# Opendigitalradio/ODR-AudioEnc

Hardware: AMD Instinct MI355X
Metric: real-time stereo DAB MP2 streams sustained (frames/s) @128 kbps/48 kHz (higher is better)
Workload: dtype f64; 1 GPU; 4096 streams/GPU x 48 kHz stereo (mode 's') x 128 kbps, psy 1, full encode (BASELINE configs[1]), 32 frames/stream/step; streams_per_gpu=4096, parallelism=streams sharded over 1 GPU(s), no data-path collective

## Files before the change

odr-audioenc_amd/csrc/mp2_psy13.h:

```cpp
#ifndef MP2_WAVE_PARTS
#error "include mp2_wave.h"
#endif

#define TL_LOGTAB(db) ((const uint64_t *)((db) + 1002))
TL_FN double tl_power_db(double e, const uint64_t *lt)
{
    return 10 * tlm_log10_pn(__builtin_fmax(e, 1E-20), lt) + TL_POWERNORM;
}
TL_FN double tl_power_db_main(double e, const uint64_t *lt, bool *near1)
{
    return 10 * tlm_log10_main_pn(__builtin_fmax(e, 1E-20), lt, near1) + TL_POWERNORM;
}
#define TL_DEFER(w) ((uint16_t *)(w).cinfo)
TL_FN void tl_power_near1(TlPsyLds &w, int pos0, int cnt)
{
    TL_LANES_BEGIN
    if (lane < cnt) {
        const int i = TL_DEFER(w)[pos0 + lane];
        const double e = w.u.fft[TL_EX(i)];
        TL_PX(w)[i] = 10 * tlm_log10_near1_pn(__builtin_fmax(e, 1E-20)) + TL_POWERNORM;
    }
    TL_LANES_END
}
#define TL_POWER_DEFER(w, flag, line_expr, ndef) do { \
// ... 245 lines not shown
    }
    TL_LANES_END
    int nlist = 0;
    if (!any_erased) {
        nlist = nconf;
        TL_LANES_BEGIN
        for (int i = lane; i < nconf; i += 64) w.tlist[i] = (int16_t)i;
        TL_LANES_END
    } else {
        PV(int, nx0); PV(int, nx1);
        TL_LANES_BEGIN L(nx0) = w.conf_nxt[lane]; L(nx1) = w.conf_nxt[64 + lane < TL_TONE_MAX ? 64 + lane : 0]; TL_LANES_END
        int i = nconf ? 0 : TL_LAST, guard = 0;
        while (i != TL_LAST && i != TL_STOP && guard++ < TL_TONE_MAX) {
            w.tlist[nlist++] = (int16_t)i;
            i = i < 64 ? TL_READLANE_I32(nx0, i) : TL_READLANE_I32(nx1, i - 64);
        }
        TL_SYNC();
    }
    TL_STAMP(sp, 3);

    const int nbands = C->p1_ncb - 1;
    {
        double *vt = w.u.fft, *vp = px;
        int nvalid = 0;
        PA(uint32_t, linfo, 8); PA(double, lrw, 8);
        TL_LANES_BEGIN
#ifndef TL_EMULATE
#pragma unroll
#endif
        for (int c8 = 0; c8 < 8; c8++) { L(linfo)[c8] = C->p1_lineinfo[64 * c8 + lane]; L(lrw)[c8] = C->p1_linerw[64 * c8 + lane]; }
        TL_LANES_END
#ifndef TL_EMULATE
#pragma unroll
#endif
        for (int base = 0; base < (TL_EXP_LEVEL >= 4 ? 0 : 512); base += 64) {
            PV(bool, ok); PV(double, tv); PV(double, pvv); PV(int, bnd);
            TL_LANES_BEGIN
            const int j = base + lane;
            const uint32_t info = L(linfo)[base >> 6];
            const int lo = (int)((info >> 8) & 0xfffu), hi = (int)(info >> 20);
            bool v = false; double t = 0, p = 0;
            if (info) {
                p = px[j];
                v = w.ptype[j] != TL_T_TONE && p != TL_DBMIN;
                t = tl_div_by(1073741824 * energy[TL_EX(j)] * (double)(j - lo), (double)(hi - lo), L(lrw)[base >> 6]);
            }
            L(ok) = v; L(tv) = t; L(pvv) = p; L(bnd) = (info && j == lo) ? (int)(info & 0xffu) : -1;
            TL_LANES_END
            const uint64_t m = TL_BALLOT(ok);
            TL_LANES_BEGIN
            const int pos = nvalid + __builtin_popcountll(m & ((1ull << lane) - 1ull));
            if (L(bnd) >= 0) w.bandoff[L(bnd)] = (int16_t)pos;
            if (L(ok)) { vt[pos] = L(tv); vp[pos] = L(pvv); }
            TL_LANES_END
            nvalid += __builtin_popcountll(m);
        }
        w.bandoff[nbands] = (int16_t)nvalid;
        TL_SYNC();
    }
    TlPsy1Ch r;
    r.nconf = nconf; r.nlist = nlist;
    r.dead_head = nconf > 0 && ((w.conf_c[0] >> 13) & 1);
    TL_DBG_TONES(nconf, r.dead_head); TL_DBG_CAND(ncand);
    return r;
}

TL_FN void tl_psy1_weights2(TlPsyLds &w, int nbands, PARG(int, r0), PARG(int, r1), PARG(double, wt))
{
    TL_LANES_BEGIN
    double weight = 0.0;
    const int band = lane & 31;
    if (band < nbands) {
        const bool second = lane >= 32;
        const double *vt = second ? w.u.fft : TL_PX(w);
        const int i0 = second ? (int)w.bandoff[band] : L(r0), i1 = second ? (int)w.bandoff[band + 1] : L(r1);
        int i = i0;
        for (; i + 16 <= i1; i += 16) {
            double t[16];
#ifndef TL_EMULATE
#pragma unroll
#endif
            for (int q = 0; q < 16; q++) t[q] = vt[i + q];
#ifndef TL_EMULATE
#pragma unroll
#endif
            for (int q = 0; q < 16; q++) weight += t[q];
        }
        for (; i < i1; i++) weight += vt[i];
    }
    L(wt) = weight;
    TL_LANES_END
}

TL_FN void tl_psy1_chain(TlPsyLds &w, const double *TL_RESTRICT db, int nbands, PARG(double, bsum), PARG(double, wt))
{
    TL_LANES_BEGIN
    double sum = TL_DBMIN, weight = 0.0;
    if (lane < nbands) {
        const double *vt = w.u.fft, *vp = TL_PX(w);
        const int i0 = w.bandoff[lane], i1 = w.bandoff[lane + 1];
        int i = i0;
        for (; i + 4 <= i1; i += 4) {
            const double p0 = vp[i], p1 = vp[i + 1], p2 = vp[i + 2], p3 = vp[i + 3];
            const double t0 = vt[i], t1 = vt[i + 1], t2 = vt[i + 2], t3 = vt[i + 3];
            sum = tl_add_db(db, p0, sum); weight += t0;
            sum = tl_add_db(db, p1, sum); weight += t1;
            sum = tl_add_db(db, p2, sum); weight += t2;
            sum = tl_add_db(db, p3, sum); weight += t3;
        }
        for (; i < i1; i++) { sum = tl_add_db(db, vp[i], sum); weight += vt[i]; }
    }
    L(bsum) = sum; L(wt) = weight;
    TL_LANES_END
}

TL_FN void tl_psy1_chain2(TlPsyLds &w, const double *TL_RESTRICT db, int nbands, PARG(int, r0), PARG(int, r1), PARG(double, bsum))
{
    TL_LANES_BEGIN
    double sum = TL_DBMIN;
    const int band = lane & 31;
    if (band < nbands) {
        const bool second = lane >= 32;
        const double *vp = second ? TL_PX(w) : w.u.fft;
        const int i0 = second ? (int)w.bandoff[band] : L(r0), i1 = second ? (int)w.bandoff[band + 1] : L(r1);
        int i = i0;
        for (; i + 8 <= i1; i += 8) {
            double p[8];
#ifndef TL_EMULATE
#pragma unroll
#endif
            for (int q = 0; q < 8; q++) p[q] = vp[i + q];
#ifndef TL_EMULATE
#pragma unroll
#endif
            for (int q = 0; q < 8; q++) sum = tl_add_db(db, p[q], sum);
        }
        for (; i + 4 <= i1; i += 4) {
            const double p0 = vp[i], p1 = vp[i + 1], p2 = vp[i + 2], p3 = vp[i + 3];
            sum = tl_add_db(db, p0, sum); sum = tl_add_db(db, p1, sum); sum = tl_add_db(db, p2, sum); sum = tl_add_db(db, p3, sum);
        }
        for (; i < i1; i++) sum = tl_add_db(db, vp[i], sum);
    }
    L(bsum) = sum;
    TL_LANES_END
}

TL_FN void tl_psy1_limits(const TlConfig *TL_RESTRICT C, int nbands, PARG(int, blo), PARG(int, bhi))
{
    TL_LANES_BEGIN
    const int b = lane < nbands ? lane : 0;
    L(blo) = C->p1_cbound[b]; L(bhi) = C->p1_cbound[b + 1];
    TL_LANES_END
}
TL_FN void tl_psy1_centres(TlPsyLds &w, int nbands, PARG(double, bsum), PARG(double, wt), PARG(int, blo), PARG(int, bhi))
{
    TL_LANES_BEGIN
    if (lane < nbands) {
        const int lo = L(blo), hi = L(bhi);
        const double sum = L(bsum), weight = L(wt);
        int centre;
        if (sum <= TL_DBMIN) centre = (hi + lo) / 2;
        else {
            double index = weight * tlm_pow10_sl(-0.1 * sum);
            centre = lo + (int)(index * (double)(hi - lo));
        }
        centre = centre < 1 ? 1 : centre > 510 ? 510 : centre;
        if (w.ptype[centre] == TL_T_TONE) { if (w.ptype[centre + 1] == TL_T_TONE) centre++; else centre--; }
        w.nsum[lane] = sum; w.ncentre[lane] = (int16_t)centre;
    }
    TL_LANES_END
}

TL_FN void tl_psy1_thresholds(TlPsyLds &w, const double *TL_RESTRICT db, const TlConfig *TL_RESTRICT C, int ch, int ntone, int nnoise, PARGA(double, rec, 4), long long *sp)
{
    TL_STAMP(sp, 5);
    TL_PRIO2(TL_PS_THR);

    TL_DBG_DUMP("psy1", ch, ntone, nnoise, TL_MK_X(w), TL_MK_BARK(w));
    const int sub = C->p1_sub;
    PV(double, tb0); PV(double, tb1); PV(double, th0); PV(double, th1); PV(int, mmn); PV(int, mmj);
    TL_LANES_BEGIN
    {
        const int k0 = 1 + 2 * lane, k1 = k0 + 1;
        const int q0 = k0 < sub ? k0 : 0, q1 = k1 < sub ? k1 : q0;
        L(tb0) = C->p1_bark[q0]; L(tb1) = C->p1_bark[q1]; L(th0) = C->p1_hear[q0]; L(th1) = C->p1_hear[q1];
        L(mmn) = C->p1_mm_n[lane & 31]; L(mmj) = C->p1_mm_j0[lane & 31];
    }
    TL_LANES_END
    TL_LANES_BEGIN
    for (int t = lane; t < ntone + nnoise; t += 64) tl_masker_consts(TL_MK4(w), TL_MK_X(w), TL_MK_BARK(w), t, t < ntone);
    TL_LANES_END
    const bool srt = ntone < 128 && nnoise < 64 && tl_maskers_sorted(TL_MK_BARK(w), ntone, nnoise);
    for (int base = 1; base < (TL_EXP_LEVEL >= 1 ? 0 : sub); base += 128) {
        TL_LANES_BEGIN
        const int k0 = base + 2 * lane, k1 = k0 + 1;
        const bool h0 = k0 < sub, h1 = k1 < sub;
        if (h0) {
            double bk0 = L(tb0), bk1 = L(tb1), hr0 = L(th0), hr1 = L(th1);
            if (base != 1) {
                bk0 = C->p1_bark[k0]; bk1 = C->p1_bark[h1 ? k1 : k0]; hr0 = C->p1_hear[k0]; hr1 = C->p1_hear[h1 ? k1 : k0];
            }
            const double blo = (bk0 < bk1 ? bk0 : bk1) - 8.0, bhi = (bk0 < bk1 ? bk1 : bk0) + 3.0;
            const TlMasker *mk = TL_MK4(w);
            const int nm = ntone + nnoise;
            int a0, a1, b0, b1;
            if (srt) tl_mask_spans_sorted<64, 32>(TL_MK_BARK(w), ntone, nnoise, blo, bhi, a0, a1, b0, b1);
            else tl_mask_spans(mk, nm, ntone, blo, bhi, a0, a1, b0, b1);
            double x0 = TL_DBMIN, x1 = TL_DBMIN;
            const int nt = a1 >= a0 ? a1 - a0 + 1 : 0, cnt = nt + (b1 >= b0 ? b1 - b0 + 1 : 0);
            int t = nt ? a0 : b0;
            TL_DBG_WALK(ch, lane, cnt);
            const TlMaskK kk = tl_mask_consts();
            for (int i = 0; i < cnt; i += 2) {
                const int tA = t, tB = tA == a1 ? b0 : tA + 1;
                t = tB == a1 ? b0 : tB + 1;
                const TlMasker *pA = &mk[tA & (TL_MASKER_MAX - 1)], *pB = &mk[tB & (TL_MASKER_MAX - 1)];
                const double bA = pA->bark, avA = pA->av, bB = pB->bark, avB = pB->av;
                const bool two = i + 1 < cnt;
                const double mA0 = tl_mask_term_w(pA, bA - bk0, avA, kk.far_hi), mA1 = tl_mask_term_w(pA, bA - bk1, avA, kk.far_hi);
                const double mB0 = tl_mask_term_w(pB, bB - bk0, avB, kk.far_hi, two), mB1 = tl_mask_term_w(pB, bB - bk1, avB, kk.far_hi, two);
                tl_add_db2_k(db, kk.k1000, x0, mA0, x1, mA1);
                tl_add_db2_k(db, kk.k1000, x0, mB0, x1, mB1);
            }
            TL_LTG(w)[k0] = tl_add_db(db, C->br_per_ch < 96 ? hr0 : hr0 - 12.0, x0);
            if (h1) TL_LTG(w)[k1] = tl_add_db(db, C->br_per_ch < 96 ? hr1 : hr1 - 12.0, x1);
        }
        TL_LANES_END
    }
    TL_STAMP(sp, 6);

    TL_LANES_BEGIN
    if (lane < C->sblimit) {
        double m;
        int n = L(mmn), j0 = L(mmj);
        if (n == 0) m = C->p1_hear[sub - 1];
        else {
            m = tl_min_rows(TL_LTG(w), j0, n, 0.0, true);
        }
        L(rec)[2 + ch] = m;
    } else if (lane < 32) L(rec)[2 + ch] = 0.0;
    TL_LANES_END
}

TL_FN void tl_psy1_back(TlPsyLds &w, const double *TL_RESTRICT db, const TlConfig *TL_RESTRICT C, int ch, const TlPsy1Ch &st, PARGA(double, rec, 4), long long *sp, bool stamp4 = true)
{
    const int nbands = C->p1_ncb - 1, nlist = st.nlist;
    int ntone = 0, nnoise = 0;
    if (stamp4) TL_STAMP(sp, 4);
    if (TL_EXP_LEVEL >= 2) { tl_psy1_thresholds(w, db, C, ch, 0, 0, rec, sp); return; }
    PV(int, ncen); PV(double, nlev); PV(int, nsh); PV(int, nsl); PV(bool, ontone);
    TL_LANES_BEGIN
    L(ncen) = lane < nbands ? (int)w.ncentre[lane] : -1 - lane;
    const double v = lane < nbands ? w.nsum[lane] : 0.0;
    L(nlev) = v; L(nsh) = (int)(uint32_t)(tl_d2u(v) >> 32); L(nsl) = (int)(uint32_t)tl_d2u(v);
    L(ontone) = lane < nbands && w.ptype[L(ncen)] == TL_T_TONE;
    TL_LANES_END
    const bool centre_on_tone = TL_BALLOT(ontone) != 0ull;
    PV(bool, shared_c);
    uint8_t *cmark = (uint8_t *)w.cinfo;
    TL_LANES_BEGIN if (lane < nbands) cmark[L(ncen)] = (uint8_t)lane; TL_LANES_END
    TL_LANES_BEGIN L(shared_c) = lane < nbands && cmark[L(ncen)] != (uint8_t)lane; TL_LANES_END
    if (TL_BALLOT(shared_c) != 0ull)
        for (int b = 1; b < nbands; b++) {
            const int cb = TL_READLANE_I32(ncen, b);
            const double vb = tl_u2d(((uint64_t)(uint32_t)TL_READLANE_I32(nsh, b) << 32) | (uint32_t)TL_READLANE_I32(nsl, b));
            TL_LANES_BEGIN if (lane < b && L(ncen) == cb) L(nlev) = vb; TL_LANES_END
        }

    {
        PV(double, nbk0); PV(double, nhear0);
        TL_LANES_BEGIN
        const int c0 = lane < nbands ? L(ncen) : 1;
        L(nbk0) = C->p1_lbark[c0]; L(nhear0) = C->p1_lhear[c0];
        TL_LANES_END
        for (int base = 0; base < nlist; base += 64) {
            PV(bool, keep); PV(double, kx); PV(double, kb); PV(int, tline); PV(int, tcc); PV(double, tbk); PV(double, thr);
            TL_LANES_BEGIN
            double x = 0; int c = -1000 - lane, cc = 0;
            if (base + lane < nlist) { const int ti = w.tlist[base + lane]; cc = w.conf_c[ti]; c = cc & 511; x = w.tone_x[ti]; }
            L(kx) = x; L(tline) = c; L(tcc) = cc;
            L(tbk) = C->p1_lbark[c < 0 ? 0 : c]; L(thr) = C->p1_lhear[c < 0 ? 0 : c];
            TL_LANES_END
            if (centre_on_tone)
                for (int b = 0; b < nbands; b++) {
                    const int cb = TL_READLANE_I32(ncen, b);
                    const double vb = tl_u2d(((uint64_t)(uint32_t)TL_READLANE_I32(nsh, b) << 32) | (uint32_t)TL_READLANE_I32(nsl, b));
                    TL_LANES_BEGIN if (L(tline) == cb) L(kx) = vb; TL_LANES_END
                }
            TL_LANES_BEGIN
            bool kp = false; double bk = 0;
            if (base + lane < nlist) {
                bk = L(tbk);
                kp = !((L(tcc) >> 13) & 1) && !(L(kx) < L(thr));
            }
            L(keep) = kp; L(kb) = bk;
            TL_LANES_END
            const uint64_t m = TL_BALLOT(keep);
            TL_LANES_BEGIN
            if ((m >> lane) & 1ull) {
                const int pos = ntone + __builtin_popcountll(m & ((1ull << lane) - 1ull));
                TL_MK_X(w)[pos] = L(kx); TL_MK_BARK(w)[pos] = L(kb);
            }
            TL_LANES_END
            ntone += __builtin_popcountll(m);
        }
        {
            PV(bool, closep);
            TL_LANES_BEGIN
            bool cl = false;
            for (int q = 1 + lane; q < ntone; q += 64) cl = cl || (TL_MK_BARK(w)[q] - TL_MK_BARK(w)[q - 1] < 0.5);
            L(closep) = cl;
            TL_LANES_END
            if (TL_BALLOT(closep) != 0ull) {
                int n = 0;
                double xi = TL_MK_X(w)[0], bi = TL_MK_BARK(w)[0];
                for (int q = 1; q < ntone; q++) {
                    const double xn = TL_MK_X(w)[q], bn = TL_MK_BARK(w)[q];
                    if (bn - bi < 0.5) {
                        if (xn > xi) { xi = xn; bi = bn; }
                    } else { TL_MK_X(w)[n] = xi; TL_MK_BARK(w)[n] = bi; n++; xi = xn; bi = bn; }
                }
                TL_MK_X(w)[n] = xi; TL_MK_BARK(w)[n] = bi; n++;
                ntone = n;
                TL_SYNC();
            }
        }
        PV(bool, keepn); PV(double, nx); PV(double, nb);
        TL_LANES_BEGIN
        bool kp = false; double x = 0, bk = 0;
        if (lane < nbands) {
            x = L(nlev); bk = L(nbk0);
            kp = !(x < L(nhear0));
        }
        L(keepn) = kp; L(nx) = x; L(nb) = bk;
        TL_LANES_END
        const uint64_t mn = TL_BALLOT(keepn);
        TL_LANES_BEGIN
        if ((mn >> lane) & 1ull) {
            const int pos = ntone + __builtin_popcountll(mn & ((1ull << lane) - 1ull));
            TL_MK_X(w)[pos] = L(nx); TL_MK_BARK(w)[pos] = L(nb);
        }
        TL_LANES_END
        nnoise = __builtin_popcountll(mn);
    }
    tl_psy1_thresholds(w, db, C, ch, ntone, nnoise, rec, sp);
}

TL_FN void tl_psy1_deadhead(TlPsyLds &w, const double *TL_RESTRICT db, const TlConfig *TL_RESTRICT C, int ch, const TlPsy1Ch &st, PARGA(double, rec, 4), long long *sp)
{
    const int nbands = C->p1_ncb - 1, nconf = st.nconf;
    const uint8_t *map = C->p1_map;
    double *px = TL_PX(w);
    int ntone = 0, nnoise = 0;
    TL_STAMP(sp, 4);
    {
        TL_LANES_BEGIN
        for (int j = lane; j < 520; j += 64) px[j] = TL_DBMIN;
        TL_LANES_END
        TL_LANES_BEGIN
        for (int i = lane; i < nconf; i += 64) { const int cc = w.conf_c[i]; if (!((cc >> 13) & 1)) px[cc & 511] = w.tone_x[i]; }
        TL_LANES_END
        TL_DBG_DUMP("deadhead", ch, 0, 0, px, px);
        int16_t *pnext = (int16_t *)w.cinfo;
        TL_LANES_BEGIN
        for (int i = lane; i < 512; i += 64) pnext[i] = TL_STOP;
        TL_LANES_END
        TL_LANES_BEGIN
        for (int i = lane; i < nconf; i += 64) {
            const int nx = w.conf_nxt[i];
            pnext[w.conf_c[i] & 511] = (int16_t)(nx >= 0 ? (w.conf_c[nx] & 511) : nx);
        }
        TL_LANES_END
        int tone = w.conf_c[0] & 511, noise = 0;
        {
            int last = TL_LAST;
            for (int i = 0; i < nbands; i++) {
                const int centre = w.ncentre[i];
                if (last == TL_LAST) noise = centre;
                else { pnext[centre] = TL_LAST; pnext[last] = (int16_t)centre; }
                px[centre] = w.nsum[i]; w.ptype[centre] = TL_T_NOISE; last = centre;
            }
        }
        {
            int i = tone, old = TL_STOP, guard = 0;
            while (i != TL_LAST && i != TL_STOP && guard++ < 600) {
                if (px[i] < C->p1_hear[map[i]]) {
                    w.ptype[i] = 0; px[i] = TL_DBMIN;
                    if (old == TL_STOP) tone = pnext[i]; else pnext[old] = pnext[i];
                } else old = i;
                i = pnext[i];
            }
            i = noise; old = TL_STOP; guard = 0;
            while (i != TL_LAST && i != TL_STOP && guard++ < 600) {
                if (px[i] < C->p1_hear[map[i]]) {
                    w.ptype[i] = 0; px[i] = TL_DBMIN;
                    if (old == TL_STOP) noise = pnext[i]; else pnext[old] = pnext[i];
                } else old = i;
                i = pnext[i];
            }
            i = tone; old = TL_STOP; guard = 0;
            while (i != TL_LAST && i != TL_STOP && guard++ < 600) {
                const int nx = pnext[i];
                if (nx == TL_LAST) break;
                if (nx == TL_STOP) break;
                if (C->p1_bark[map[nx]] - C->p1_bark[map[i]] < 0.5) {
                    if (px[nx] > px[i]) {
                        if (old == TL_STOP) tone = nx; else pnext[old] = (int16_t)nx;
                        w.ptype[i] = 0; px[i] = TL_DBMIN; i = nx;
                    } else {
                        w.ptype[nx] = 0; px[nx] = TL_DBMIN;
                        pnext[i] = pnext[nx]; old = i;
                    }
                } else { old = i; i = nx; }
            }
            guard = 0;
            for (int t = tone; t != TL_LAST && t != TL_STOP && ntone < TL_MASKER_MAX - 32 && guard++ < 600; t = pnext[t]) {
                TL_MK_X(w)[ntone] = px[t]; TL_MK_BARK(w)[ntone] = C->p1_bark[map[t]]; ntone++;
            }
            guard = 0;
            for (int t = noise; t != TL_LAST && t != TL_STOP && ntone + nnoise < TL_MASKER_MAX && guard++ < 600; t = pnext[t]) {
                TL_MK_X(w)[ntone + nnoise] = px[t]; TL_MK_BARK(w)[ntone + nnoise] = C->p1_bark[map[t]]; nnoise++;
            }
        }
        TL_SYNC();
    }
    tl_psy1_thresholds(w, db, C, ch, ntone, nnoise, rec, sp);
}

TL_FN void tl_psy1_finish(TlPsyLds &w, const double *TL_RESTRICT db, const TlConfig *TL_RESTRICT C, int ch, const TlPsy1Ch &st, PARGA(double, rec, 4), long long *sp)
{
    const int nbands = C->p1_ncb - 1;
    PV(double, wt); PV(double, bsum); PV(int, blo); PV(int, bhi);
    tl_psy1_limits(C, nbands, blo, bhi);
    TL_PRIO(1); tl_psy1_chain(w, db, nbands, bsum, wt); TL_PRIO(0);
    tl_psy1_centres(w, nbands, bsum, wt, blo, bhi);
    if (st.dead_head) tl_psy1_deadhead(w, db, C, ch, st, rec, sp); else tl_psy1_back(w, db, C, ch, st, rec, sp);
}
TL_FN void tl_psy1(TlPsyLds &w, const TlTables *TL_RESTRICT T, const double *TL_RESTRICT db,
                   const TlConfig *TL_RESTRICT C, const TlPcmView &pv, int ch, PARGA(double, rec, 4), long long *sp)
{
    const TlPsy1Ch st = tl_psy1_front(w, T, db, C, pv, ch, rec, sp);
    tl_psy1_finish(w, db, C, ch, st, rec, sp);
}

TL_FN void tl_psy1_stereo(TlPsyLds &w, const TlTables *TL_RESTRICT T, const double *TL_RESTRICT db,
                          const TlConfig *TL_RESTRICT C, const TlPcmView &pv, PARGA(double, rec, 4), long long *sp)
{
    const int nbands = C->p1_ncb - 1;
    long long *sp0 = sp ? sp + 8 : nullptr, *sp1 = sp ? sp + 16 : nullptr;
    const TlPsy1Ch s0 = tl_psy1_front(w, T, db, C, pv, 0, rec, sp0);
    if (s0.dead_head) {
        tl_psy1_finish(w, db, C, 0, s0, rec, sp0);
        tl_psy1(w, T, db, C, pv, 1, rec, sp1);
        return;
    }
    PV(int, r0); PV(int, r1);
    PA(double, pvp, 8); PA(double, pvt, 8); PV(int, pcc); PV(int, ptl); PV(double, ptx0); PV(double, ptx1);
    TL_LANES_BEGIN
    L(r0) = lane < nbands ? (int)w.bandoff[lane] : 0; L(r1) = lane < nbands ? (int)w.bandoff[lane + 1] : 0;
    const double *vp = TL_PX(w), *vt = w.u.fft;
#ifndef TL_EMULATE
#pragma unroll
#endif
    for (int k = 0; k < 8; k++) L(pvp)[k] = lane + 64 * k < 504 ? vp[lane + 64 * k] : 0.0;
#ifndef TL_EMULATE
#pragma unroll
#endif
    for (int k = 0; k < 8; k++) L(pvt)[k] = lane + 64 * k < 504 ? vt[lane + 64 * k] : 0.0;
    const int hi = 64 + lane < TL_TONE_MAX ? 64 + lane : 0;
    L(pcc) = (int)((uint32_t)(uint16_t)w.conf_c[lane] | ((uint32_t)(uint16_t)w.conf_c[hi] << 16));
    L(ptl) = (int)((uint32_t)(uint16_t)w.tlist[lane] | ((uint32_t)(uint16_t)w.tlist[hi] << 16));
    L(ptx0) = w.tone_x[lane]; L(ptx1) = w.tone_x[hi];
    TL_LANES_END
    const TlPsy1Ch s1 = tl_psy1_front(w, T, db, C, pv, 1, rec, sp1);
    PV(double, bsum); PV(double, wt); PV(int, blo); PV(int, bhi);
    tl_psy1_limits(C, nbands, blo, bhi);
    if (s1.dead_head) {
        tl_psy1_finish(w, db, C, 1, s1, rec, sp1);
        TL_LANES_BEGIN
#ifndef TL_EMULATE
#pragma unroll
#endif
        for (int k = 0; k < 8; k++) if (lane + 64 * k < 504) { TL_PX(w)[lane + 64 * k] = L(pvp)[k]; w.u.fft[lane + 64 * k] = L(pvt)[k]; }
        if (lane <= nbands) w.bandoff[lane] = (int16_t)(lane < nbands ? L(r0) : 0);
        TL_LANES_END
        {
            const int last_end = TL_READLANE_I32(r1, nbands - 1);
            TL_LANES_BEGIN if (lane == 0) w.bandoff[nbands] = (int16_t)last_end; TL_LANES_END
        }
        TL_PRIO(1); tl_psy1_chain(w, db, nbands, bsum, wt); TL_PRIO(0);
    } else {
        TL_LANES_BEGIN
#ifndef TL_EMULATE
#pragma unroll
#endif
        for (int k = 0; k < 8; k++) if (lane + 64 * k < 504) {
            const double v = TL_PX(w)[lane + 64 * k];
            TL_PX(w)[lane + 64 * k] = L(pvt)[k]; L(pvt)[k] = v;
        }
        TL_LANES_END
        if (TL_EXP_LEVEL < 3) tl_psy1_weights2(w, nbands, r0, r1, wt);
        TL_LANES_BEGIN
#ifndef TL_EMULATE
#pragma unroll
#endif
        for (int k = 0; k < 8; k++) if (lane + 64 * k < 504) { w.u.fft[lane + 64 * k] = L(pvp)[k]; TL_PX(w)[lane + 64 * k] = L(pvt)[k]; }
        TL_LANES_END
        TL_STAMP(sp1, 4);
        if (TL_EXP_LEVEL < 3) { TL_PRIO(1); tl_psy1_chain2(w, db, nbands, r0, r1, bsum); TL_PRIO(0); }
        TL_STAMP(sp0, 4);
        PV(double, bsum1); PV(double, wt1);
#ifdef TL_EMULATE
        for (int lane = 0; lane < 64; ++lane) { bsum1[lane] = bsum[(lane + 32) & 63]; wt1[lane] = wt[(lane + 32) & 63]; }
#else
        bsum1 = __shfl(bsum, (int)((threadIdx.x + 32u) & 63u), 64);
        wt1 = __shfl(wt, (int)((threadIdx.x + 32u) & 63u), 64);
#endif
        if (TL_EXP_LEVEL < 3) tl_psy1_centres(w, nbands, bsum1, wt1, blo, bhi);
        tl_psy1_back(w, db, C, 1, s1, rec, sp1, false);
    }
    TL_LANES_BEGIN
    for (int i = lane; i < 520; i += 64) w.ptype[i] = 0;
    const int hi = 64 + lane < TL_TONE_MAX ? 64 + lane : 0;
    w.conf_c[lane] = (int16_t)(L(pcc) & 0xffff); w.tlist[lane] = (int16_t)(L(ptl) & 0xffff); w.tone_x[lane] = L(ptx0);
    if (64 + lane < TL_TONE_MAX) { w.conf_c[hi] = (int16_t)((uint32_t)L(pcc) >> 16); w.tlist[hi] = (int16_t)((uint32_t)L(ptl) >> 16); w.tone_x[hi] = L(ptx1); }
    TL_LANES_END
    TL_LANES_BEGIN
    for (int i = lane; i < s0.nconf; i += 64) { const int cc = w.conf_c[i]; if (!((cc >> 13) & 1)) w.ptype[cc & 511] = TL_T_TONE; }
    TL_LANES_END
    if (TL_EXP_LEVEL < 3) tl_psy1_centres(w, nbands, bsum, wt, blo, bhi);
    tl_psy1_back(w, db, C, 0, s0, rec, sp0, s1.dead_head);
}

TL_FN int tl_psy3_front(TlPsyLds &w, const TlTables *TL_RESTRICT T, const double *TL_RESTRICT db,
                   const TlConfig *TL_RESTRICT C, const TlPcmView &pv, int ch, PARGA(double, rec, 4), long long *sp)
{
    const double *energy = w.u.fft;
    double *px = TL_PX(w);
    const double *bark = C->p3_bark, *ath = C->p3_ath;
    TL_PRIO2(TL_PS_FHT);
    TL_STAMP(sp, 0);
    tl_psy_spectrum(w, T, pv, ch, sp);
    TL_STAMP(sp, 1);
    TL_PRIO2(TL_PS_POW);

    PA(double, pxa, 8);
    int ndef = 0;
    for (int h = 0; h < 2; h++) {
        PV(bool, n0); PV(bool, n1); PV(bool, n2); PV(bool, n3);
        TL_LANES_BEGIN
        {
            double e[4], v[4];
            bool nr[4];
#ifndef TL_EMULATE
#pragma unroll
#endif
            for (int q = 0; q < 4; q++) { const int i = lane + 64 * (4 * h + q); e[q] = energy[TL_EX(i == 0 ? 512 : i)]; }
#ifndef TL_EMULATE
#pragma unroll
#endif
            for (int q = 0; q < 4; q++) v[q] = tl_power_db_main(e[q], TL_LOGTAB(db), &nr[q]);
#ifndef TL_EMULATE
#pragma unroll
#endif
            for (int q = 0; q < 4; q++) { const int i = lane + 64 * (4 * h + q); px[i == 0 ? 512 : i] = v[q]; }
            if (h == 0 && lane == 0) px[0] = 0.0;
            L(n0) = nr[0]; L(n1) = nr[1]; L(n2) = nr[2]; L(n3) = nr[3];
        }
        TL_LANES_END
        TL_POWER_DEFER(w, n0, (h == 0 && lane == 0) ? 512 : lane + 256 * h, ndef);
        TL_POWER_DEFER(w, n1, lane + 256 * h + 64, ndef);
        TL_POWER_DEFER(w, n2, lane + 256 * h + 128, ndef);
        TL_POWER_DEFER(w, n3, lane + 256 * h + 192, ndef);
        while (ndef >= 64) { ndef -= 64; TL_DBG_NEAR1_FULL(); tl_power_near1(w, ndef, 64); }
    }
    if (ndef) tl_power_near1(w, 0, ndef);
    TL_LANES_BEGIN
#ifndef TL_EMULATE
#pragma unroll
#endif
    for (int k = 0; k < 8; k++) { const int i = lane + 64 * k; L(pxa)[k] = i == 0 ? TL_DBMIN : px[i]; }
    TL_LANES_END
#ifndef TL_EMULATE
#pragma unroll
#endif
    for (int it = 0; it < 8; it++) {
        PV(double, pxv); PV(double, pxm);
        TL_LANES_BEGIN L(pxv) = L(pxa)[it]; TL_LANES_END
        TL_ROW16_MAX_F64(pxm, pxv);
        PV(double, xm);
        TL_LANES_BEGIN L(xm) = TL_DBMIN < L(pxm) ? L(pxm) : TL_DBMIN; TL_LANES_END
        TL_LANES_BEGIN
        {
            const double v = TL_OTHER(xm, , 16 * (lane & 3) + 15);
            if (lane < 32 && (lane >> 2) == it) L(rec)[ch] = v;
        }
        TL_LANES_END
    }
    TL_PRIO2(1);
    int ncand = 0;
    tl_cand_chunk<2, true>(w, 0, ncand);
    tl_cand_chunk<3, true>(w, 1, ncand);
    for (int c8 = 2; c8 < 4; c8++) tl_cand_chunk<6, true>(w, c8, ncand);
    for (int c8 = 4; c8 < 8; c8++) tl_cand_chunk<12, true>(w, c8, ncand);
    TL_STAMP(sp, 2);
    int nconf = 0;
    {
        int R = -1;
        for (int kb = 0; kb < ncand; kb += 64) {
        PV(int, ck); PV(int, csr); PV(int, clf); PV(bool, act); PV(bool, dep);
        TL_LANES_BEGIN
        const bool in = kb + lane < ncand;
        const uint32_t info = w.cinfo[in ? kb + lane : 0];
        const uint32_t pinfo = w.cinfo[in && kb + lane > 0 ? kb + lane - 1 : 0];
        L(ck) = (int)(info & 511u); L(csr) = (int)(info >> 21);
        L(clf) = (int)tl_cand_left<true>(px, L(ck), L(csr), px[L(ck)]);
        L(act) = in;
        L(dep) = in && kb + lane > 0 && L(ck) - (int)(pinfo & 511u) < (int)(pinfo >> 21) + L(csr) + 1;
        TL_LANES_END
        for (;;) {
            PV(bool, okv);
            TL_LANES_BEGIN
            const int k = L(ck), sr = L(csr);
            const int hi_j = sr < k - R - 1 ? sr : k - R - 1;
            const uint32_t orig = hi_j >= 2 ? (1u << (hi_j - 1)) - 1u : 0u;
            L(okv) = L(act) && k > R && !((uint32_t)L(clf) & orig);
            TL_LANES_END
            const uint64_t m = TL_BALLOT(okv);
            if (m == 0ull) break;
            const int wl = __builtin_ctzll(m);
            PV(bool, depact);
            TL_LANES_BEGIN L(depact) = L(dep) && L(act) && lane > wl; TL_LANES_END
            const uint64_t dm = TL_BALLOT(depact);
            const uint64_t batch = m & (dm ? (1ull << __builtin_ctzll(dm)) - 1ull : ~0ull);
            const int nb = __builtin_popcountll(batch), wlast = 63 - __builtin_clzll(batch);
            const int i0 = nconf, Rold = R;
            TL_LANES_BEGIN
            if ((batch >> lane) & 1ull) {
                const int i = i0 + __builtin_popcountll(batch & ((1ull << lane) - 1ull));
                if (i < TL_TONE_MAX) w.conf_c[i] = (int16_t)(L(ck) | ((lane == wl && L(ck) - 1 <= Rold) ? (1 << 12) : 0));
            }
            TL_LANES_END
            nconf = i0 + nb < TL_TONE_MAX ? i0 + nb : (i0 < TL_TONE_MAX ? TL_TONE_MAX : i0);
            R = TL_READLANE_I32(ck, wlast) + TL_READLANE_I32(csr, wlast);
            TL_LANES_BEGIN L(act) = L(act) && lane > wlast; TL_LANES_END
            TL_DBG_ROUND();
        }
        }
        TL_SYNC();
    }
    TL_LANES_BEGIN
    for (int i = lane; i < nconf; i += 64) {
        const int cc = w.conf_c[i], k = cc & 511;
        const double temp = tl_add_db(db, (cc >> 12) & 1 ? TL_DBMIN : px[k - 1], px[k]);
        w.tone_x[i] = tl_add_db(db, temp, px[k + 1]);
    }
    TL_LANES_END
    TL_LANES_BEGIN
    for (int i = lane; i < nconf; i += 64) {
        const int k = w.conf_c[i] & 511, sr = tl_run_psy3(k);
        double *pb = px + (k - 12);
#define TL_ERASE3(j) do { pb[12 - (j)] = TL_DBMIN; pb[12 + (j)] = TL_DBMIN; } while (0)
        pb[12] = TL_DBMIN; TL_ERASE3(1); TL_ERASE3(2);
// ... 327 lines not shown
```

odr-audioenc_amd/csrc/mp2_wave.h:

```cpp
#pragma once
#include "mp2_types.h"
#include "tl_libm.h"
#include <math.h>
#include <stddef.h>

#ifdef TL_EMULATE
#define TL_FN static inline
#define TL_LANES_BEGIN for (int lane = 0; lane < 64; ++lane) {
#define TL_LANES_END }
#define TL_SYNC() ((void)0)
#define PV(T, name) T name[64]
#define PA(T, name, n) T name[64][n]
#define L(name) name[lane]
#define PARG(T, name) T (&name)[64]
#define PARGA(T, name, n) T (&name)[64][n]
#define TL_OTHER(name, idx, src) name[src] idx
#define TL_ATOMIC_OR(p, v) (*(p) |= (v))
TL_FN uint64_t tlh_ballot(const bool (&p)[64]) { uint64_t m = 0; for (int i = 0; i < 64; i++) if (p[i]) m |= 1ull << i; return m; }
TL_FN uint64_t tlh_min_u64(const uint64_t (&v)[64]) { uint64_t m = v[0]; for (int i = 1; i < 64; i++) if (v[i] < m) m = v[i]; return m; }
TL_FN int tlh_sum_i32(const int (&v)[64]) { int s = 0; for (int i = 0; i < 64; i++) s += v[i]; return s; }
TL_FN uint32_t tlh_xor_u32(const uint32_t (&v)[64]) { uint32_t s = 0; for (int i = 0; i < 64; i++) s ^= v[i]; return s; }
TL_FN void tlh_exscan_i32(int (&d)[64], const int (&v)[64]) { int s = 0; for (int i = 0; i < 64; i++) { d[i] = s; s += v[i]; } }
TL_FN int tlh_argmin_u64(const uint64_t (&v)[64])
{
// ... 80 lines not shown
    int v = (int)x;
    v ^= __builtin_amdgcn_update_dpp(0, v, 0x111, 0xf, 0xf, false);
    v ^= __builtin_amdgcn_update_dpp(0, v, 0x112, 0xf, 0xf, false);
    v ^= __builtin_amdgcn_update_dpp(0, v, 0x114, 0xf, 0xf, false);
    v ^= __builtin_amdgcn_update_dpp(0, v, 0x118, 0xf, 0xf, false);
    v ^= __builtin_amdgcn_update_dpp(0, v, 0x142, 0xa, 0xf, false);
    v ^= __builtin_amdgcn_update_dpp(0, v, 0x143, 0xc, 0xf, false);
    return (uint32_t)__builtin_amdgcn_readlane(v, 63);
}
TL_FN int tld_sum_i32(int v) { return __builtin_amdgcn_readlane(tld_incl_scan_i32(v), 63); }
TL_FN int tld_exscan_i32(int v) { return tld_incl_scan_i32(v) - v; }
TL_FN int tld_argmin_u64(uint64_t v)
{
    const uint32_t hi = (uint32_t)(v >> 32), lo = (uint32_t)v;
    const uint32_t mhi = tld_min_u32(hi);
    uint64_t m = (uint64_t)__ballot(hi == mhi);
    if (__builtin_popcountll(m) > 1) {
        const uint32_t mlo = tld_min_u32(hi == mhi ? lo : 0xffffffffu);
        if ((mhi & mlo) == 0xffffffffu) return -1;
        m = (uint64_t)__ballot(hi == mhi && lo == mlo);
    } else if (mhi == 0xffffffffu && (uint32_t)__builtin_amdgcn_readlane((int)lo, __builtin_ctzll(m)) == 0xffffffffu) return -1;
    const uint64_t even = m & 0x5555555555555555ull;
    return __builtin_ctzll(even ? even : m);
}
TL_FN double tld_row16_max_f64(double v)
{
#pragma unroll
    for (int sh = 1; sh <= 8; sh <<= 1) {
        const uint64_t u = tl_d2u(v);
        const int ctl = 0x110 | sh;
        uint32_t lo, hi;
        switch (sh) {
        case 1: lo = (uint32_t)__builtin_amdgcn_update_dpp((int)(uint32_t)u, (int)(uint32_t)u, 0x111, 0xf, 0xf, false); hi = (uint32_t)__builtin_amdgcn_update_dpp((int)(uint32_t)(u >> 32), (int)(uint32_t)(u >> 32), 0x111, 0xf, 0xf, false); break;
        case 2: lo = (uint32_t)__builtin_amdgcn_update_dpp((int)(uint32_t)u, (int)(uint32_t)u, 0x112, 0xf, 0xf, false); hi = (uint32_t)__builtin_amdgcn_update_dpp((int)(uint32_t)(u >> 32), (int)(uint32_t)(u >> 32), 0x112, 0xf, 0xf, false); break;
        case 4: lo = (uint32_t)__builtin_amdgcn_update_dpp((int)(uint32_t)u, (int)(uint32_t)u, 0x114, 0xf, 0xf, false); hi = (uint32_t)__builtin_amdgcn_update_dpp((int)(uint32_t)(u >> 32), (int)(uint32_t)(u >> 32), 0x114, 0xf, 0xf, false); break;
        default: lo = (uint32_t)__builtin_amdgcn_update_dpp((int)(uint32_t)u, (int)(uint32_t)u, 0x118, 0xf, 0xf, false); hi = (uint32_t)__builtin_amdgcn_update_dpp((int)(uint32_t)(u >> 32), (int)(uint32_t)(u >> 32), 0x118, 0xf, 0xf, false); break;
        }
        (void)ctl;
        const double o = tl_u2d(((uint64_t)hi << 32) | lo);
        v = v < o ? o : v;
    }
    return v;
}
#define TL_ROW16_MAX_F64(dst, src) dst = tld_row16_max_f64(src)
TL_FN uint32_t tld_incl_xscan_u32(uint32_t x)
{
    int v = (int)x;
    v ^= __builtin_amdgcn_update_dpp(0, v, 0x111, 0xf, 0xf, false);
    v ^= __builtin_amdgcn_update_dpp(0, v, 0x112, 0xf, 0xf, false);
    v ^= __builtin_amdgcn_update_dpp(0, v, 0x114, 0xf, 0xf, false);
    v ^= __builtin_amdgcn_update_dpp(0, v, 0x118, 0xf, 0xf, false);
    v ^= __builtin_amdgcn_update_dpp(0, v, 0x142, 0xa, 0xf, false);
    v ^= __builtin_amdgcn_update_dpp(0, v, 0x143, 0xc, 0xf, false);
    return (uint32_t)v;
}
#define TL_WAVE_INCL_XSCAN_U32(dst, src) dst = tld_incl_xscan_u32(src)
TL_FN uint32_t tld_par_min_u32(uint32_t v)
{
    uint32_t t;
    t = (uint32_t)__builtin_amdgcn_update_dpp((int)v, (int)v, 0x122, 0xf, 0xf, false); v = t < v ? t : v;
    t = (uint32_t)__builtin_amdgcn_update_dpp((int)v, (int)v, 0x124, 0xf, 0xf, false); v = t < v ? t : v;
    t = (uint32_t)__builtin_amdgcn_update_dpp((int)v, (int)v, 0x128, 0xf, 0xf, false); v = t < v ? t : v;
    const auto r = __builtin_amdgcn_permlane16_swap(v, v, false, false); v = r[0] < r[1] ? r[0] : r[1];
    const auto q = __builtin_amdgcn_permlane32_swap(v, v, false, false); v = q[0] < q[1] ? q[0] : q[1];
    return v;
}
TL_FN uint64_t tld_par_min_u64(uint64_t v)
{
    const uint32_t hi = (uint32_t)(v >> 32), lo = (uint32_t)v;
    const uint32_t mhi = tld_par_min_u32(hi);
    const uint32_t mlo = tld_par_min_u32(hi == mhi ? lo : 0xffffffffu);
    return ((uint64_t)mhi << 32) | mlo;
}
TL_FN int tld_par_sum_i32(int v)
{
    v += __builtin_amdgcn_update_dpp(v, v, 0x122, 0xf, 0xf, false);
    v += __builtin_amdgcn_update_dpp(v, v, 0x124, 0xf, 0xf, false);
    v += __builtin_amdgcn_update_dpp(v, v, 0x128, 0xf, 0xf, false);
    const auto r = __builtin_amdgcn_permlane16_swap((unsigned)v, (unsigned)v, false, false); v = (int)(r[0] + r[1]);
    const auto q = __builtin_amdgcn_permlane32_swap((unsigned)v, (unsigned)v, false, false); v = (int)(q[0] + q[1]);
    return v;
}
#define TL_PAR_MIN_U64(dst, src) dst = tld_par_min_u64(src)
#define TL_PAR_SUM_I32(dst, src) dst = tld_par_sum_i32(src)
#define TL_BALLOT(name) ((uint64_t)__ballot(name))
#define TL_SWAP1_U64(dst, src) dst = tl_d2u(tld_swap1_f64(tl_u2d(src)))
#define TL_WAVE_ARGMIN_U64(name) tld_argmin_u64(name)
#define TL_WAVE_MIN_U64(name) tld_min_u64(name)
#define TL_WAVE_SUM_I32(name) tld_sum_i32(name)
#define TL_WAVE_XOR_U32(name) tld_xor_u32(name)
#define TL_WAVE_EXSCAN_I32(dst, src) dst = tld_exscan_i32(src)
#define TL_UNI_I(x) __builtin_amdgcn_readfirstlane(x)
#define TL_READLANE_I32(name, l) __builtin_amdgcn_readlane(name, l)
#define TL_RESTRICT __restrict__
#define TL_SELECT(c, a, b) (__builtin_unpredictable(c) ? (a) : (b))
#define TL_KEEP(x) asm volatile("" : : "v"(x))
typedef double tl_f64x2 __attribute__((ext_vector_type(2)));
#define TL_LD2(p, a, b) do { const tl_f64x2 v_ = *(const tl_f64x2 *)(p); (a) = v_.x; (b) = v_.y; } while (0)
#if defined(__HIP_DEVICE_COMPILE__)
typedef const __attribute__((address_space(4))) struct TlLaunch *TlKArg;
#else
typedef const struct TlLaunch *TlKArg;
#endif
#define TL_KARG TlKArg
#define TL_LAUNDER(p) asm volatile("" : "+s"(p))
#define TL_TIE(p, v) asm volatile("" : "+s"(p), "+v"(v))
#define TL_PIN(x) asm volatile("" : "+v"(x))
#endif

#ifndef TL_PRIO_CHAIN
#define TL_PRIO_CHAIN 3
#endif
#ifndef TL_PS_FHT
#define TL_PS_FHT 0
#endif
#ifndef TL_PS_THR
#define TL_PS_THR 1
#endif
#ifndef TL_PS_FB
#define TL_PS_FB 0
#endif
#ifndef TL_PS_Q
#define TL_PS_Q 0
#endif
#ifndef TL_PS_POW
#define TL_PS_POW 1
#endif
#ifndef TL_PRIO_SERIAL
#define TL_PRIO_SERIAL 2
#endif
#ifdef TL_EMULATE
#define TL_PRIO(n) ((void)0)
#define TL_PRIO2(n) ((void)0)
#else
#define TL_PRIO(n) do { if (TL_PRIO_CHAIN) __builtin_amdgcn_s_setprio((n) ? TL_PRIO_CHAIN : TL_PRIO_SERIAL); } while (0)
#define TL_PRIO2(n) do { if (TL_PRIO_SERIAL) __builtin_amdgcn_s_setprio((n) ? TL_PRIO_SERIAL : 0); } while (0)
#endif
#ifdef TL_EMULATE
#define TL_STAMP(sp, k) ((void)0)
#else
#define TL_STAMP(sp, k) do { if (sp) { long long t_ = (long long)__builtin_amdgcn_s_memtime(); if ((threadIdx.x & 63u) == 0) (sp)[k] = t_; } } while (0)
#endif

#if defined(TL_EMULATE) && defined(TL_DEBUG_DUMP)
#include <stdio.h>
#include <stdlib.h>
#define TL_DBG_DUMP(tag, ch, nt, nn, x, b) do { if (getenv("TL_DUMP")) { printf("%s ch%d ntone %d nnoise %d:", tag, ch, nt, nn); \
    for (int i_ = 0; i_ < (nt) + (nn); i_++) printf(" (%.17g,%.6f)", (x)[i_], (b)[i_]); printf("\n"); } } while (0)
#define TL_DBG_WALK(ch, lane, cnt) do { if (getenv("TL_DUMP_WALK")) printf("walk ch%d lane %d cnt %d\n", ch, lane, cnt); } while (0)
static long tl_dbg_rounds = 0, tl_dbg_tones = 0, tl_dbg_deadheads = 0, tl_dbg_fronts = 0, tl_dbg_cands = 0;
#define TL_DBG_CAND(n) (tl_dbg_cands += (n))
#define TL_DBG_ROUND() (tl_dbg_rounds++)
#define TL_DBG_TONES(n, dh) (tl_dbg_tones += (n), tl_dbg_deadheads += (dh) ? 1 : 0, tl_dbg_fronts++)
#else
#define TL_DBG_DUMP(tag, ch, nt, nn, x, b) ((void)0)
#define TL_DBG_WALK(ch, lane, cnt) ((void)0)
#define TL_DBG_ROUND() ((void)0)
#define TL_DBG_TONES(n, dh) ((void)0)
#define TL_DBG_CAND(n) ((void)0)
#endif
#ifndef TL_EXP_LEVEL
#define TL_EXP_LEVEL 0
#endif
#ifndef TL_ENC_LEVEL
#define TL_ENC_LEVEL 0
#endif
#ifndef TL_P2_LEVEL
#define TL_P2_LEVEL 0
#endif
#ifndef TL_P2_SUB
#define TL_P2_SUB 0
#endif
#ifndef TL_P3_NOTAIL
#define TL_P3_NOTAIL 0
#endif
#define TL_DBMIN (-200.0)
#define TL_POWERNORM 90.3090
#define TL_T_NOISE 10
#define TL_T_TONE 20
#define TL_LAST (-1)
#define TL_STOP (-100)

#define TL_CAND_MAX 256
#ifndef TL_FB_BATCH_MAIN
#define TL_FB_BATCH_MAIN 6
#endif
#define TL_PSY_EXT 5
#define TL_TONE_MAX 77
#define TL_MASKER_MAX 128
#define TL_FFT_WORDS (513 + 520)
#define TL_PX(w) ((w).u.fft + 513)
#define TL_EX(i) ((i) ^ (((i) >> 4) & 15))
#define TL_YP_ROW 18
struct TlMainLds {
    static constexpr int kFbBatch = TL_FB_BATCH_MAIN;
    union alignas(16) {
        struct { int16_t pcm[2][TL_HIST + 1152]; } fbk;
        uint32_t frame[2][TL_MAX_FRAME_WORDS + 2];
    } u;
    alignas(16) double yp[TL_FB_BATCH_MAIN][TL_YP_ROW * 3 + 16];
    double smr[2][32];
    double psy_m[2][32];
    int16_t ncentre[32];
    uint8_t scf[2][3][32];
    uint8_t jscale[3][32];
    uint8_t scfsi[2][32];
    uint8_t balloc[2][32];
    uint8_t minidx[2][32];
    uint8_t xpad[TL_MAX_XPAD];
    typedef double (*YpRows)[TL_YP_ROW * 3 + 16];
#ifdef TL_EMULATE
    YpRows yp_rows() { return yp; }
#else
    __device__ YpRows yp_rows() { return yp; }
#endif
};
struct alignas(16) TlPsy2Lds {
    struct { double fft[1024]; } u;
    double px[536];
};
struct TlPsyLds {
    struct { double fft[TL_FFT_WORDS]; } u;
    double tone_x[TL_TONE_MAX];
    double nsum[32];
    uint32_t cinfo[TL_CAND_MAX];
    int16_t conf_c[TL_TONE_MAX];
    int16_t conf_nxt[TL_TONE_MAX];
    int16_t tlist[TL_TONE_MAX];
    int16_t ncentre[32];
    int16_t bandoff[40];
    uint8_t ptype[520];
};
#define TL_MK_X(w) ((w).u.fft)
#define TL_MK_BARK(w) ((w).u.fft + TL_MASKER_MAX)
#define TL_LTG(w) ((w).u.fft + 2 * TL_MASKER_MAX)
struct TlMasker { double bark, av, g, c17, n; };
#define TL_MK4(w) ((TlMasker *)((w).u.fft + 2 * TL_MASKER_MAX + 136))
static_assert(2 * TL_MASKER_MAX + 136 + 5 * TL_MASKER_MAX <= TL_FFT_WORDS, "masker records fit the transform buffer");



#ifdef TL_EMULATE
static long tl_emu_near1_full = 0;
#define TL_DBG_NEAR1_FULL() (tl_emu_near1_full++)
#else
#define TL_DBG_NEAR1_FULL() ((void)0)
#endif

#define MP2_WAVE_PARTS 1
#include "mp2_dbsum.h"
#include "mp2_fht.h"
#include "mp2_psy13.h"
#include "mp2_psy24.h"
#include "mp2_fb.h"
#include "mp2_alloc.h"
#include "mp2_pack.h"
#include "mp2_units.h"
#undef MP2_WAVE_PARTS
```

Measured before the change: 36.04 million frames/s.

## Process both stereo channels' psy1 centre and decimation steps in one wave

Adds a paired path for the psy-model-1 back half: when both channels' tone lists fit within 32 entries, the centre search and masker decimation for channel 0 and channel 1 run together, with lanes 0-31 and 32-63 each handling one channel. Channel 0's state is staged in a spare region of the transform buffer. The aim is to replace two serial per-channel passes that each used only half the wavefront, which shortens the serial critical path. In exchange it adds LDS staging copies, a more complex merge loop, and a fallback for longer lists. Debug counters are also added for the emulator build.

```diff
diff --git a/odr-audioenc_amd/csrc/mp2_psy13.h b/odr-audioenc_amd/csrc/mp2_psy13.h
--- a/odr-audioenc_amd/csrc/mp2_psy13.h
+++ b/odr-audioenc_amd/csrc/mp2_psy13.h
@@ -421,6 +421,13 @@
     L(blo) = C->p1_cbound[b]; L(bhi) = C->p1_cbound[b + 1];
     TL_LANES_END
 }
+TL_FN void tl_psy1_limits2(const TlConfig *TL_RESTRICT C, int nbands, PARG(int, blo), PARG(int, bhi))
+{
+    TL_LANES_BEGIN
+    const int b = (lane & 31) < nbands ? (lane & 31) : 0;
+    L(blo) = C->p1_cbound[b]; L(bhi) = C->p1_cbound[b + 1];
+    TL_LANES_END
+}
 TL_FN void tl_psy1_centres(TlPsyLds &w, int nbands, PARG(double, bsum), PARG(double, wt), PARG(int, blo), PARG(int, bhi))
 {
     TL_LANES_BEGIN
@@ -437,6 +444,27 @@
         if (w.ptype[centre] == TL_T_TONE) { if (w.ptype[centre + 1] == TL_T_TONE) centre++; else centre--; }
         w.nsum[lane] = sum; w.ncentre[lane] = (int16_t)centre;
     }
+    TL_LANES_END
+}
+TL_FN void tl_psy1_centres2(TlPsyLds &w, int nbands, PARG(double, bsum), PARG(double, wt), PARG(int, blo), PARG(int, bhi), PARG(int, ncen), PARG(bool, ontone))
+{
+    TL_LANES_BEGIN
+    int centre = -1 - lane;
+    bool ont = false;
+    if ((lane & 31) < nbands) {
+        const uint8_t *pt = lane >= 32 ? w.ptype : TL_P1B_PTYPE(w);
+        const int lo = L(blo), hi = L(bhi);
+        const double sum = L(bsum), weight = L(wt);
+        if (sum <= TL_DBMIN) centre = (hi + lo) / 2;
+        else {
+            double index = weight * tlm_pow10_sl(-0.1 * sum);
+            centre = lo + (int)(index * (double)(hi - lo));
+        }
+        centre = centre < 1 ? 1 : centre > 510 ? 510 : centre;
+        if (pt[centre] == TL_T_TONE) { TL_DBG_BACK(2); if (pt[centre + 1] == TL_T_TONE) centre++; else centre--; }
+        ont = pt[centre] == TL_T_TONE;
+    }
+    L(ncen) = centre; L(ontone) = ont;
     TL_LANES_END
 }
 
@@ -615,6 +643,129 @@
     tl_psy1_thresholds(w, db, C, ch, ntone, nnoise, rec, sp);
 }
 
+struct TlPsy1Mk2 { int ntone0, nnoise0, ntone1, nnoise1; };
+TL_FN TlPsy1Mk2 tl_psy1_decimate2(TlPsyLds &w, const TlConfig *TL_RESTRICT C, int nbands, int nl0, int nl1, PARG(int, tl0),
+                                  PARG(double, bsum), PARG(int, ncen), PARG(bool, ontone))
+{
+    PV(double, nlev); PV(int, nsh); PV(int, nsl);
+    TL_LANES_BEGIN
+    const double v = (lane & 31) < nbands ? L(bsum) : 0.0;
+    L(nlev) = v; L(nsh) = (int)(uint32_t)(tl_d2u(v) >> 32); L(nsl) = (int)(uint32_t)tl_d2u(v);
+    TL_LANES_END
+    const bool centre_on_tone = TL_BALLOT(ontone) != 0ull;
+    if (centre_on_tone) TL_DBG_BACK(6);
+    PV(bool, shared_c);
+    uint8_t *cmark = (uint8_t *)w.cinfo;
+    TL_LANES_BEGIN if ((lane & 31) < nbands) cmark[((lane >> 5) << 9) + L(ncen)] = (uint8_t)(lane & 31); TL_LANES_END
+    TL_LANES_BEGIN L(shared_c) = (lane & 31) < nbands && cmark[((lane >> 5) << 9) + L(ncen)] != (uint8_t)(lane & 31); TL_LANES_END
+    if (TL_BALLOT(shared_c) != 0ull) {
+        TL_DBG_BACK(3);
+        for (int b = 1; b < nbands; b++) {
+            const int cb0 = TL_READLANE_I32(ncen, b), cb1 = TL_READLANE_I32(ncen, 32 + b);
+            const double vb0 = tl_u2d(((uint64_t)(uint32_t)TL_READLANE_I32(nsh, b) << 32) | (uint32_t)TL_READLANE_I32(nsl, b));
+            const double vb1 = tl_u2d(((uint64_t)(uint32_t)TL_READLANE_I32(nsh, 32 + b) << 32) | (uint32_t)TL_READLANE_I32(nsl, 32 + b));
+            TL_LANES_BEGIN if ((lane & 31) < b && L(ncen) == (lane >= 32 ? cb1 : cb0)) L(nlev) = lane >= 32 ? vb1 : vb0; TL_LANES_END
+        }
+    }
+    TlPsy1Mk2 r;
+    PV(double, nbk0); PV(double, nhear0);
+    TL_LANES_BEGIN
+    const int c0 = (lane & 31) < nbands ? L(ncen) : 1;
+    L(nbk0) = C->p1_lbark[c0]; L(nhear0) = C->p1_lhear[c0];
+    TL_LANES_END
+    {
+        PV(bool, keep); PV(double, kx); PV(double, kb); PV(int, tline); PV(int, tcc); PV(double, tbk); PV(double, thr); PV(bool, inl);
+        TL_LANES_BEGIN
+        const bool second = lane >= 32;
+        const int k = lane & 31;
+        const bool in = k < (second ? nl1 : nl0);
+        double x = 0; int c = -1000 - lane, cc = 0;
+        if (in) {
+            const int ti = second ? (int)w.tlist[k] : (int)(int16_t)(L(tl0) & 0xffff);
+            const int16_t *cf = second ? w.conf_c : TL_P1B_CONF_C(w);
+            const double *tx = second ? w.tone_x : TL_P1B_TONE_X(w);
+            cc = cf[ti]; c = cc & 511; x = tx[ti];
+        }
+        L(kx) = x; L(tline) = c; L(tcc) = cc; L(inl) = in;
+        L(tbk) = C->p1_lbark[c < 0 ? 0 : c]; L(thr) = C->p1_lhear[c < 0 ? 0 : c];
+        TL_LANES_END
+        if (centre_on_tone)
+            for (int b = 0; b < nbands; b++) {
+                const int cb0 = TL_READLANE_I32(ncen, b), cb1 = TL_READLANE_I32(ncen, 32 + b);
+                const double vb0 = tl_u2d(((uint64_t)(uint32_t)TL_READLANE_I32(nsh, b) << 32) | (uint32_t)TL_READLANE_I32(nsl, b));
+                const double vb1 = tl_u2d(((uint64_t)(uint32_t)TL_READLANE_I32(nsh, 32 + b) << 32) | (uint32_t)TL_READLANE_I32(nsl, 32 + b));
+                TL_LANES_BEGIN if (L(tline) == (lane >= 32 ? cb1 : cb0)) L(kx) = lane >= 32 ? vb1 : vb0; TL_LANES_END
+            }
+        TL_LANES_BEGIN
+        bool kp = false; double bk = 0;
+        if (L(inl)) {
+            bk = L(tbk);
+            kp = !((L(tcc) >> 13) & 1) && !(L(kx) < L(thr));
+        }
+        L(keep) = kp; L(kb) = bk;
+        TL_LANES_END
+        const uint64_t m = TL_BALLOT(keep);
+        TL_LANES_BEGIN
+        if ((m >> lane) & 1ull) {
+            const bool second = lane >= 32;
+            const int pos = __builtin_popcountll(m & ((1ull << lane) - 1ull) & (second ? ~0xffffffffull : 0xffffffffull));
+            (second ? TL_MK_X(w) : TL_P1B_MKX(w))[pos] = L(kx); (second ? TL_MK_BARK(w) : TL_P1B_MKBARK(w))[pos] = L(kb);
+        }
+        TL_LANES_END
+        r.ntone0 = __builtin_popcountll(m & 0xffffffffull); r.ntone1 = __builtin_popcountll(m >> 32);
+    }
+    {
+        PV(bool, closep);
+        TL_LANES_BEGIN
+        const bool second = lane >= 32;
+        const int q = 1 + (lane & 31);
+        const double *bk = second ? TL_MK_BARK(w) : TL_P1B_MKBARK(w);
+        L(closep) = q < (second ? r.ntone1 : r.ntone0) && (bk[q] - bk[q - 1] < 0.5);
+        TL_LANES_END
+        const uint64_t cm = TL_BALLOT(closep);
+        if (cm != 0ull) {
+            const bool do0 = (cm & 0xffffffffull) != 0ull, do1 = (cm >> 32) != 0ull;
+            double *X0 = TL_P1B_MKX(w), *B0 = TL_P1B_MKBARK(w), *X1 = TL_MK_X(w), *B1 = TL_MK_BARK(w);
+            const int t0 = do0 ? r.ntone0 : 0, t1 = do1 ? r.ntone1 : 0;
+            int n0 = 0, n1 = 0;
+            double xi0 = X0[0], bi0 = B0[0], xi1 = X1[0], bi1 = B1[0];
+            for (int q = 1; q < (t0 > t1 ? t0 : t1); q++) {
+                if (q < t0) {
+                    const double xn = X0[q], bn = B0[q];
+                    if (bn - bi0 < 0.5) {
+                        if (xn > xi0) { xi0 = xn; bi0 = bn; }
+                    } else { X0[n0] = xi0; B0[n0] = bi0; n0++; xi0 = xn; bi0 = bn; }
+                }
+                if (q < t1) {
+                    const double xn = X1[q], bn = B1[q];
+                    if (bn - bi1 < 0.5) {
+                        if (xn > xi1) { xi1 = xn; bi1 = bn; }
+                    } else { X1[n1] = xi1; B1[n1] = bi1; n1++; xi1 = xn; bi1 = bn; }
+                }
+            }
+            if (do0) { X0[n0] = xi0; B0[n0] = bi0; r.ntone0 = n0 + 1; }
+            if (do1) { X1[n1] = xi1; B1[n1] = bi1; r.ntone1 = n1 + 1; }
+            TL_SYNC();
+        }
+    }
+    {
+        PV(bool, keepn);
+        TL_LANES_BEGIN
+        L(keepn) = (lane & 31) < nbands && !(L(nlev) < L(nhear0));
+        TL_LANES_END
+        const uint64_t mn = TL_BALLOT(keepn);
+        TL_LANES_BEGIN
+        if ((mn >> lane) & 1ull) {
+            const bool second = lane >= 32;
+            const int pos = (second ? r.ntone1 : r.ntone0) + __builtin_popcountll(mn & ((1ull << lane) - 1ull) & (second ? ~0xffffffffull : 0xffffffffull));
+            (second ? TL_MK_X(w) : TL_P1B_MKX(w))[pos] = L(nlev); (second ? TL_MK_BARK(w) : TL_P1B_MKBARK(w))[pos] = L(nbk0);
+        }
+        TL_LANES_END
+        r.nnoise0 = __builtin_popcountll(mn & 0xffffffffull); r.nnoise1 = __builtin_popcountll(mn >> 32);
+    }
+    return r;
+}
+
 TL_FN void tl_psy1_deadhead(TlPsyLds &w, const double *TL_RESTRICT db, const TlConfig *TL_RESTRICT C, int ch, const TlPsy1Ch &st, PARGA(double, rec, 4), long long *sp)
 {
     const int nbands = C->p1_ncb - 1, nconf = st.nconf;
@@ -719,6 +870,7 @@
     long long *sp0 = sp ? sp + 8 : nullptr, *sp1 = sp ? sp + 16 : nullptr;
     const TlPsy1Ch s0 = tl_psy1_front(w, T, db, C, pv, 0, rec, sp0);
     if (s0.dead_head) {
+        TL_DBG_BACK(4);
         tl_psy1_finish(w, db, C, 0, s0, rec, sp0);
         tl_psy1(w, T, db, C, pv, 1, rec, sp1);
         return;
@@ -743,8 +895,9 @@
     TL_LANES_END
     const TlPsy1Ch s1 = tl_psy1_front(w, T, db, C, pv, 1, rec, sp1);
     PV(double, bsum); PV(double, wt); PV(int, blo); PV(int, bhi);
-    tl_psy1_limits(C, nbands, blo, bhi);
+    tl_psy1_limits2(C, nbands, blo, bhi);
     if (s1.dead_head) {
+        TL_DBG_BACK(5);
         tl_psy1_finish(w, db, C, 1, s1, rec, sp1);
         TL_LANES_BEGIN
 #ifndef TL_EMULATE
@@ -778,6 +931,36 @@
         TL_STAMP(sp1, 4);
         if (TL_EXP_LEVEL < 3) { TL_PRIO(1); tl_psy1_chain2(w, db, nbands, r0, r1, bsum); TL_PRIO(0); }
         TL_STAMP(sp0, 4);
+        if (s0.nlist <= TL_P1B_LIST && s1.nlist <= TL_P1B_LIST) {
+            TL_DBG_BACK(0);
+            PV(int, ncen); PV(bool, ontone);
+            TlPsy1Mk2 mk = {0, 0, 0, 0};
+            if (TL_EXP_LEVEL < 3) {
+                TL_LANES_BEGIN
+                ((double *)TL_P1B_PTYPE(w))[lane] = 0.0;
+                if (lane == 0) ((double *)TL_P1B_PTYPE(w))[64] = 0.0;
+                const int hi = 64 + lane < TL_TONE_MAX ? 64 + lane : 0;
+                TL_P1B_CONF_C(w)[lane] = (int16_t)(L(pcc) & 0xffff); TL_P1B_TONE_X(w)[lane] = L(ptx0);
+                if (64 + lane < TL_TONE_MAX) { TL_P1B_CONF_C(w)[hi] = (int16_t)((uint32_t)L(pcc) >> 16); TL_P1B_TONE_X(w)[hi] = L(ptx1); }
+                TL_LANES_END
+                TL_LANES_BEGIN
+                if (lane < s0.nconf) { const int cc = L(pcc) & 0xffff; if (!((cc >> 13) & 1)) TL_P1B_PTYPE(w)[cc & 511] = TL_T_TONE; }
+                if (64 + lane < s0.nconf) { const int cc = (int)((uint32_t)L(pcc) >> 16); if (!((cc >> 13) & 1)) TL_P1B_PTYPE(w)[cc & 511] = TL_T_TONE; }
+                TL_LANES_END
+                tl_psy1_centres2(w, nbands, bsum, wt, blo, bhi, ncen, ontone);
+                if (TL_EXP_LEVEL < 2) mk = tl_psy1_decimate2(w, C, nbands, s0.nlist, s1.nlist, ptl, bsum, ncen, ontone);
+            }
+            tl_psy1_thresholds(w, db, C, 1, mk.ntone1, mk.nnoise1, rec, sp1);
+            TL_LANES_BEGIN
+            if (lane < mk.ntone0 + mk.nnoise0) {
+                const double x = TL_P1B_MKX(w)[lane], bk = TL_P1B_MKBARK(w)[lane];
+                TL_MK_X(w)[lane] = x; TL_MK_BARK(w)[lane] = bk;
+            }
+            TL_LANES_END
+            tl_psy1_thresholds(w, db, C, 0, mk.ntone0, mk.nnoise0, rec, sp0);
+            return;
+        }
+        TL_DBG_BACK(1);
         PV(double, bsum1); PV(double, wt1);
 #ifdef TL_EMULATE
         for (int lane = 0; lane < 64; ++lane) { bsum1[lane] = bsum[(lane + 32) & 63]; wt1[lane] = wt[(lane + 32) & 63]; }
diff --git a/odr-audioenc_amd/csrc/mp2_wave.h b/odr-audioenc_amd/csrc/mp2_wave.h
--- a/odr-audioenc_amd/csrc/mp2_wave.h
+++ b/odr-audioenc_amd/csrc/mp2_wave.h
@@ -256,7 +256,11 @@
 #define TL_DBG_CAND(n) (tl_dbg_cands += (n))
 #define TL_DBG_ROUND() (tl_dbg_rounds++)
 #define TL_DBG_TONES(n, dh) (tl_dbg_tones += (n), tl_dbg_deadheads += (dh) ? 1 : 0, tl_dbg_fronts++)
-#else
+static long tl_dbg_back[7] = {0, 0, 0, 0, 0, 0, 0};
+#define TL_DBG_BACK(k) (tl_dbg_back[k]++)
+extern "C" __attribute__((weak, visibility("default"))) void emu_back_stats(long *out) { for (int i = 0; i < 7; i++) out[i] = tl_dbg_back[i]; }
+#else
+#define TL_DBG_BACK(k) ((void)0)
 #define TL_DBG_DUMP(tag, ch, nt, nn, x, b) ((void)0)
 #define TL_DBG_WALK(ch, lane, cnt) ((void)0)
 #define TL_DBG_ROUND() ((void)0)
@@ -341,6 +345,15 @@
 struct TlMasker { double bark, av, g, c17, n; };
 #define TL_MK4(w) ((TlMasker *)((w).u.fft + 2 * TL_MASKER_MAX + 136))
 static_assert(2 * TL_MASKER_MAX + 136 + 5 * TL_MASKER_MAX <= TL_FFT_WORDS, "masker records fit the transform buffer");
+#define TL_P1B_LIST 32
+#define TL_P1B_BASE 700
+#define TL_P1B_MKX(w) ((w).u.fft + TL_P1B_BASE)
+#define TL_P1B_MKBARK(w) ((w).u.fft + TL_P1B_BASE + 64)
+#define TL_P1B_TONE_X(w) ((w).u.fft + TL_P1B_BASE + 128)
+#define TL_P1B_PTYPE(w) ((uint8_t *)((w).u.fft + TL_P1B_BASE + 128 + TL_TONE_MAX))
+#define TL_P1B_CONF_C(w) ((int16_t *)((w).u.fft + TL_P1B_BASE + 128 + TL_TONE_MAX + 65))
+static_assert(TL_P1B_LIST + 27 <= 64 && 2 * TL_MASKER_MAX + 136 + 5 * (TL_P1B_LIST + 27) <= TL_P1B_BASE, "channel 1's masker records end below channel 0's records");
+static_assert(TL_P1B_BASE + 128 + TL_TONE_MAX + 65 + (2 * TL_TONE_MAX + 7) / 8 <= TL_FFT_WORDS, "channel 0's records fit the transform buffer");
 
 
 
```

Result: faster. 36.44 million frames/s, median of 6 (+1.1%).
